# hby1320/pytorch_object_detection

Hardware: AMD Instinct MI355X
Metric: images/sec HISFCOS-R50 640x640 inference (higher is better)
Workload: dtype f32

## Files before the change

pytorch_object_detection_amd/csrc/fd_conv.hip:

```cpp
#include "fd_conv_common.h"

template <int WGM, int WGN, int TM, int TN, bool STEM, bool SB, int TAG, bool SPLIT, bool GATE = false, bool GNS = false, bool H1 = false, bool GEMM = false, bool DUAL = false,
          bool RUP = false>
__global__ __launch_bounds__(WGM * WGN * 64, (TM * TN == 4) ? ((SPLIT || WGM * WGN == 8) ? 2 : (SB ? 3 : 1)) : 1)
void conv_igemm_kernel(ConvArgs a) {
    constexpr int BM = WGM * TM * 32, BN = WGN * TN * 32;
    constexpr int NT = WGM * WGN * 64;
    constexpr int RPP = NT / 8;
    constexpr int AP = BM / RPP, BP = BN / RPP;
    extern __shared__ __attribute__((aligned(16))) char smem[];
    constexpr int NBUF = SB ? 1 : 2;
    float* As = reinterpret_cast<float*>(smem);
    float* Bs = As + NBUF * BM * 32;
    _Float16* Hs = reinterpret_cast<_Float16*>(smem);
    constexpr int HSTG = (BM + BN) * 64;

    const int tid = threadIdx.x, lane = tid & 63, wave = tid >> 6;
    const int wm = wave / WGN, wn = wave % WGN;

    const int nblk = a.mtiles * a.ntiles;
    int bid = blockIdx.x;
    {
        const int q = nblk >> 3, r = nblk & 7, xcd = bid & 7, idx = bid >> 3;
        bid = (xcd < r ? xcd * (q + 1) : r * (q + 1) + (xcd - r) * q) + idx;
    }
    const int mt = bid / a.ntiles, nt = bid - mt * a.ntiles;
    const int m0 = mt * BM, n0 = nt * BN;

    const int lrow = tid >> 3, chunk = tid & 7;
    constexpr unsigned OOB = 0xC0000000u;
    const int esh = (H1 && a.x16) ? 1 : 2;
    const __amdgpu_buffer_rsrc_t xrsrc = __builtin_amdgcn_make_buffer_rsrc((void*)a.x, (short)0, (int)a.x_bytes, 0x00020000);
    const __amdgpu_buffer_rsrc_t wrsrc = __builtin_amdgcn_make_buffer_rsrc((void*)a.w, (short)0, (int)a.w_bytes, 0x00020000);
    unsigned a_off[AP];
    int a_wcs[AP], a_hi0[AP], a_wi0[AP], a_H[AP], a_W[AP];
    const float* g_row[GATE ? AP : 1];
    const long gate_bo = GATE && a.gate_b ? (long)(a.gate_b - a.gate) : 0;
#pragma unroll
    for (int i = 0; i < AP; ++i) {
        const int m = m0 + lrow + RPP * i;
        if (GATE) {
            const int mm = min(m, a.M - 1);
            int sg = 0;
#pragma unroll
            for (int t = 1; t < FD_MAX_SEG; ++t)
                if (t < a.nseg && mm >= a.m_out[t]) sg = t;
            const int img = sg * a.gate_batch + (mm - a.m_out[sg]) / (a.Ho[sg] * a.Wo[sg]);
            g_row[i] = a.gate + (size_t)img * a.gate_cs + chunk * 4;
        }
        if constexpr (GEMM) {
            if (a.is_gemm) {
                a_off[i] = (m < a.M) ? ((unsigned)m * (unsigned)a.x_cs + (unsigned)(a.x_co + chunk * 4)) << esh : OOB;
                a_wcs[i] = 0; a_hi0[i] = 0; a_wi0[i] = 0; a_H[i] = 1; a_W[i] = 1;
                continue;
            }
        }
        if (a.is_gemm) {
            a_off[i] = ((unsigned)m * (unsigned)a.x_cs + (unsigned)(a.x_co + chunk * 4)) << esh;
            a_wcs[i] = 0; a_hi0[i] = 0; a_wi0[i] = 0; a_H[i] = (m < a.M) ? 1 : 0; a_W[i] = 1;
            continue;
        }
        int s = 0;
#pragma unroll
        for (int t = 1; t < FD_MAX_SEG; ++t)
            if (t < a.nseg && m >= a.m_out[t]) s = t;
        const int Ho = a.Ho[s], Wo = a.Wo[s], H = a.H[s], W = a.W[s];
        const int local = m - a.m_out[s];
        const int hw = Ho * Wo;
        const int n = local / hw;
        const int rem = local - n * hw;
        const int ho = rem / Wo, wo = rem - ho * Wo;
        a_hi0[i] = ho * a.stride - a.pad;
        a_wi0[i] = wo * a.stride - a.pad;
        a_H[i] = (m < a.M) ? H : 0;
        a_W[i] = W;
        a_wcs[i] = (W * a.x_cs) << esh;
        a_off[i] = ((unsigned)(a.m_in[s] + n * H * W + a_hi0[i] * W + a_wi0[i]) * (unsigned)a.x_cs +
                    (unsigned)(a.x_co + chunk * 4)) << esh;
        if constexpr (GEMM) { if (m >= a.M) a_off[i] = OOB; }
    }
    unsigned a2_off[DUAL ? AP : 1];
    const __amdgpu_buffer_rsrc_t x2rsrc = __builtin_amdgcn_make_buffer_rsrc((void*)(DUAL ? a.x2 : a.x), (short)0, (int)(DUAL ? a.x2_bytes : 0u), 0x00020000);
    if constexpr (DUAL) {
#pragma unroll
        for (int i = 0; i < AP; ++i) {
            const int m = m0 + lrow + RPP * i;
            const int hw = a.Ho[0] * a.Wo[0];
            const int n = m / hw, rem = m - n * hw;
            const int ho = rem / a.Wo[0], wo = rem - ho * a.Wo[0];
            const unsigned row2 = (unsigned)((n * a.x2_H + ho * a.x2_stride) * a.x2_W + wo * a.x2_stride);
            a2_off[i] = (m < a.M) ? (row2 * (unsigned)a.x2_cs + (unsigned)(a.x2_co + chunk * 4)) * 4u : OOB;
        }
    }
    unsigned b_off[BP];
#pragma unroll
    for (int j = 0; j < BP; ++j) {
        const int n = n0 + lrow + RPP * j;
        b_off[j] = (n < a.Cout && !(H1 && (chunk & 4))) ? ((unsigned)n * (unsigned)a.Kpacked + (unsigned)(chunk * 4)) * 4u : OOB;
    }

    float4 ra[AP], rb[BP], rg[GATE ? AP : 1], rgb[GATE ? AP : 1];
    auto ld_x = [&](unsigned voff, int soff) -> float4 {
        if (H1 && a.x16) {
            const f32x2 v = __builtin_bit_cast(f32x2, __builtin_amdgcn_raw_buffer_load_b64(xrsrc, (int)voff, soff, 0));
            return make_float4(v.x, v.y, 0.f, 0.f);
        }
        return __builtin_bit_cast(float4, __builtin_amdgcn_raw_buffer_load_b128(xrsrc, (int)voff, soff, 0));
    };
    int ld_cc = 0, ld_r = 0, ld_q = 0;
    auto load_tile = [&](int kt) {
        if constexpr (GEMM) {
            const int kb = kt * 128;
            const int kbx = kt << (5 + esh);
            if (GATE) {
#pragma unroll
                for (int i = 0; i < AP; ++i) {
                    rg[i] = *reinterpret_cast<const float4*>(g_row[i] + kt * 32);
                    if (a.gate_b) rgb[i] = *reinterpret_cast<const float4*>(g_row[i] + gate_bo + kt * 32);
                }
            }
            if (DUAL && kt >= a.kt2) {
                const int kb2 = (kt - a.kt2) * 128;
#pragma unroll
                for (int i = 0; i < AP; ++i) ra[i] = __builtin_bit_cast(float4, __builtin_amdgcn_raw_buffer_load_b128(x2rsrc, (int)a2_off[DUAL ? i : 0], kb2, 0));
            } else {
#pragma unroll
                for (int i = 0; i < AP; ++i) ra[i] = ld_x(a_off[i], kbx);
            }
#pragma unroll
            for (int j = 0; j < BP; ++j) rb[j] = __builtin_bit_cast(float4, __builtin_amdgcn_raw_buffer_load_b128(wrsrc, (int)b_off[j], kb, 0));
            return;
        }
        int dr, dq;
        unsigned dbytes;
        bool c_ok = true;
        if (STEM) { dr = kt; dq = 0; dbytes = 0; }
        else {
            dr = ld_r * a.dil;
            dq = ld_q * a.dil;
            dbytes = (unsigned)(dq * a.x_cs + ld_cc * 32) << esh;
            c_ok = ld_cc * 32 + chunk * 4 < a.Cin;
            if (GATE) {
#pragma unroll
                for (int i = 0; i < AP; ++i) {
                    rg[i] = c_ok ? *reinterpret_cast<const float4*>(g_row[i] + ld_cc * 32) : make_float4(0.f, 0.f, 0.f, 0.f);
                    if (a.gate_b) rgb[i] = c_ok ? *reinterpret_cast<const float4*>(g_row[i] + gate_bo + ld_cc * 32) : make_float4(0.f, 0.f, 0.f, 0.f);
                }
            }
            if (++ld_q == a.KW) { ld_q = 0; if (++ld_r * a.KW == a.ntaps) { ld_r = 0; ++ld_cc; } }
        }
#pragma unroll
        for (int i = 0; i < AP; ++i) {
            const int hi = a_hi0[i] + dr, wi = a_wi0[i] + dq + (STEM ? chunk : 0);
            bool ok = (unsigned)hi < (unsigned)a_H[i] && (unsigned)wi < (unsigned)a_W[i] && c_ok;
            if (STEM) ok = ok && (chunk < 7);
            const unsigned off = a_off[i] + (unsigned)__mul24(dr, a_wcs[i]) + dbytes;
            ra[i] = ld_x(ok ? off : OOB, 0);
        }
        const unsigned kb = (unsigned)kt * 128u;
#pragma unroll
        for (int j = 0; j < BP; ++j)
            rb[j] = __builtin_bit_cast(float4, __builtin_amdgcn_raw_buffer_load_b128(wrsrc, (int)(b_off[j] + kb), 0, 0));
    };
    auto store_tile = [&](int buf) {
        if constexpr (SPLIT) {
            _Float16* Ahi = Hs + buf * HSTG;
            _Float16* Alo = Ahi + BM * 32;
            _Float16* Bhi = Alo + BM * 32;
            _Float16* Blo = Bhi + BN * 32;
#pragma unroll
            for (int i = 0; i < AP; ++i) {
                const int row = lrow + RPP * i;
                const f32x4 v = {ra[i].x, ra[i].y, ra[i].z, ra[i].w};
                h4 hi = __builtin_convertvector(v, h4);
                if (H1 && a.x16) hi = fd_h4_bits(ra[i].x, ra[i].y);
                const int off = row * 32 + ((((chunk >> 1) ^ ((row >> 2) & 3)) << 3) | ((chunk & 1) << 2));
                *reinterpret_cast<h4*>(Ahi + off) = hi;
                if constexpr (!H1) {
                    const f32x4 rem = (v - __builtin_convertvector(hi, f32x4)) * FD_SPLIT_SCALE;
                    const h4 lo = __builtin_convertvector(rem, h4);
                    *reinterpret_cast<h4*>(Alo + off) = lo;
                }
            }
#pragma unroll
            for (int j = 0; j < BP; ++j) {
                const int row = lrow + RPP * j;
                if (!H1 || !(chunk & 4)) *reinterpret_cast<float4*>(((chunk & 4) ? Blo : Bhi) + lds_off_h(row, chunk & 3)) = rb[j];
            }
        } else {
#pragma unroll
            for (int i = 0; i < AP; ++i) {
                if (GATE) {
                    if (a.gate_b) {
                        float4 t = make_float4(fmaf(ra[i].x, rg[i].x, rgb[i].x), fmaf(ra[i].y, rg[i].y, rgb[i].y),
                                               fmaf(ra[i].z, rg[i].z, rgb[i].z), fmaf(ra[i].w, rg[i].w, rgb[i].w));
                        if (a.gate_act == FD_ACT_RELU) {
                            t.x = fmaxf(t.x, 0.f); t.y = fmaxf(t.y, 0.f); t.z = fmaxf(t.z, 0.f); t.w = fmaxf(t.w, 0.f);
                        } else if (a.gate_act == FD_ACT_SILU) {
                            t.x *= __builtin_amdgcn_rcpf(1.0f + __expf(-t.x)); t.y *= __builtin_amdgcn_rcpf(1.0f + __expf(-t.y));
                            t.z *= __builtin_amdgcn_rcpf(1.0f + __expf(-t.z)); t.w *= __builtin_amdgcn_rcpf(1.0f + __expf(-t.w));
                        }
                        ra[i] = t;
                    } else { ra[i].x *= rg[i].x; ra[i].y *= rg[i].y; ra[i].z *= rg[i].z; ra[i].w *= rg[i].w; }
                }
                *reinterpret_cast<float4*>(As + buf * BM * 32 + lds_off(lrow + RPP * i, chunk)) = ra[i];
            }
#pragma unroll
            for (int j = 0; j < BP; ++j)
                *reinterpret_cast<float4*>(Bs + buf * BN * 32 + lds_off(lrow + RPP * j, chunk)) = rb[j];
        }
    };

    f32x16 acc[TM][TN];
    f32x16 cor[SPLIT ? TM : 1][SPLIT ? TN : 1];
#pragma unroll
    for (int i = 0; i < TM; ++i)
#pragma unroll
        for (int j = 0; j < TN; ++j)
#pragma unroll
            for (int e = 0; e < 16; ++e) {
                acc[i][j][e] = 0.f;
                if constexpr (SPLIT) cor[i][j][e] = 0.f;
            }

    const int l31 = lane & 31, lh = lane >> 5;
    const int kt0 = blockIdx.y * a.kt_per;
    const int kt1 = min(a.KT, kt0 + a.kt_per);
    if (!STEM) {
        ld_cc = kt0 / a.ntaps;
        const int tap0 = kt0 - ld_cc * a.ntaps;
        ld_r = tap0 / a.KW;
        ld_q = tap0 - ld_r * a.KW;
    }
    float* const ybase = a.y + (size_t)blockIdx.y * a.slice_stride;
    auto mfma_tile = [&](int buf) {
        if constexpr (SPLIT) {
            const _Float16* Ahi = Hs + buf * HSTG + (wm * TM * 32) * 32;
            const _Float16* Alo = Ahi + BM * 32;
            const _Float16* Bhi = Hs + buf * HSTG + 2 * BM * 32 + (wn * TN * 32) * 32;
            const _Float16* Blo = Bhi + BN * 32;
#pragma unroll
            for (int ks = 0; ks < 2; ++ks) {
                h8 ah[TM], al[TM], bh[TN], bl[TN];
#pragma unroll
                for (int i = 0; i < TM; ++i) {
                    ah[i] = *reinterpret_cast<const h8*>(Ahi + lds_off_h(i * 32 + l31, 2 * ks + lh));
                    if constexpr (!H1) al[i] = *reinterpret_cast<const h8*>(Alo + lds_off_h(i * 32 + l31, 2 * ks + lh));
                }
#pragma unroll
                for (int j = 0; j < TN; ++j) {
                    bh[j] = *reinterpret_cast<const h8*>(Bhi + lds_off_h(j * 32 + l31, 2 * ks + lh));
                    if constexpr (!H1) bl[j] = *reinterpret_cast<const h8*>(Blo + lds_off_h(j * 32 + l31, 2 * ks + lh));
                }
#pragma unroll
                for (int i = 0; i < TM; ++i)
#pragma unroll
                    for (int j = 0; j < TN; ++j) {
                        acc[i][j] = __builtin_amdgcn_mfma_f32_32x32x16_f16(ah[i], bh[j], acc[i][j], 0, 0, 0);
                        if constexpr (!H1) {
                            cor[i][j] = __builtin_amdgcn_mfma_f32_32x32x16_f16(ah[i], bl[j], cor[i][j], 0, 0, 0);
                            cor[i][j] = __builtin_amdgcn_mfma_f32_32x32x16_f16(al[i], bh[j], cor[i][j], 0, 0, 0);
                        }
                    }
            }
        } else {
        const float* Ab = As + buf * BM * 32 + (wm * TM * 32) * 32;
            const float* Bb = Bs + buf * BN * 32 + (wn * TN * 32) * 32;
                __builtin_amdgcn_s_setprio(1);
#pragma unroll
            for (int s = 0; s < 4; ++s) {
                float4 fa[TM], fb[TN];
    #pragma unroll
                for (int i = 0; i < TM; ++i) fa[i] = *reinterpret_cast<const float4*>(Ab + lds_off(i * 32 + l31, 2 * s + lh));
    #pragma unroll
                for (int j = 0; j < TN; ++j) fb[j] = *reinterpret_cast<const float4*>(Bb + lds_off(j * 32 + l31, 2 * s + lh));
    #pragma unroll
                for (int i = 0; i < TM; ++i)
    #pragma unroll
                    for (int j = 0; j < TN; ++j) {
                        acc[i][j] = __builtin_amdgcn_mfma_f32_32x32x2f32(fa[i].x, fb[j].x, acc[i][j], 0, 0, 0);
                        acc[i][j] = __builtin_amdgcn_mfma_f32_32x32x2f32(fa[i].y, fb[j].y, acc[i][j], 0, 0, 0);
                        acc[i][j] = __builtin_amdgcn_mfma_f32_32x32x2f32(fa[i].z, fb[j].z, acc[i][j], 0, 0, 0);
                        acc[i][j] = __builtin_amdgcn_mfma_f32_32x32x2f32(fa[i].w, fb[j].w, acc[i][j], 0, 0, 0);
                    }
            }
            __builtin_amdgcn_s_setprio(0);
        }
    };
    load_tile(kt0);
    store_tile(0);
    __syncthreads();
    for (int kt = kt0; kt < kt1 - 1; ++kt) {
        const int buf = SB ? 0 : ((kt - kt0) & 1);
        load_tile(kt + 1);
        mfma_tile(buf);
        if (SB) __syncthreads();
        store_tile(SB ? 0 : (buf ^ 1));
        __syncthreads();
    }
#include "fd_conv_res_prefetch.inc"
    mfma_tile(SB ? 0 : ((kt1 - 1 - kt0) & 1));
    __syncthreads();

#define FD_EPI_RES_PREFETCHED
#include "fd_conv_epilogue.inc"
#undef FD_EPI_RES_PREFETCHED
}

__global__ __launch_bounds__(256) void splitk_reduce_kernel(ConvArgs a, const float* __restrict__ ws, int nslice, int ldw,
                                                             long slab) {
    const int q4 = ldw >> 2;
    const long total = (long)a.M * q4;
    for (long i = (long)blockIdx.x * 256 + threadIdx.x; i < total; i += (long)gridDim.x * 256) {
        const long m = i / q4;
        const int nn = (int)(i - m * q4) * 4;
        float4 v = *reinterpret_cast<const float4*>(ws + m * ldw + nn);
        for (int s = 1; s < nslice; ++s) {
            const float4 u = *reinterpret_cast<const float4*>(ws + s * slab + m * ldw + nn);
            v.x += u.x; v.y += u.y; v.z += u.z; v.w += u.w;
        }
        float o[4] = {v.x, v.y, v.z, v.w};
        float prm = a.seg_param[0];
        if (a.act == FD_ACT_EXP) {
#pragma unroll
            for (int t = 1; t < FD_MAX_SEG; ++t)
                prm = (t < a.nseg && m >= a.m_out[t]) ? a.seg_param[t] : prm;
        }
#pragma unroll
        for (int e = 0; e < 4; ++e) {
            const int n = nn + e;
            if (n >= a.Cout) continue;
            float r = o[e] * (a.scale ? a.scale[n] : 1.0f) + (a.shift ? a.shift[n] : 0.0f);
            const size_t mo = (size_t)out_row(a, (int)m);
            if (a.res) {
                const float rv = a.res16 ? (float)reinterpret_cast<const _Float16*>(a.res)[mo * a.res_cs + a.res_co + n] : a.res[mo * a.res_cs + a.res_co + n];
                r = a.res_mask ? (rv > 0.f ? r : 0.f) : r + rv;
            }
            const float ov = fd_act(r, n >= a.act_c0 ? a.act : FD_ACT_NONE, prm);
            if (a.y16) reinterpret_cast<_Float16*>(a.y)[mo * a.y_cs + a.y_co + n] = (_Float16)ov;
            else a.y[mo * a.y_cs + a.y_co + n] = ov;
        }
    }
}

int fd_launch_splitk_reduce(const ConvArgs& orig, const float* ws, int nslice, int ldw, long slab, hipStream_t stream) {
    long g = ((long)orig.M * (ldw >> 2) + 255) / 256;
    if (g > 16384) g = 16384;
    hipLaunchKernelGGL(splitk_reduce_kernel, dim3((unsigned)g), dim3(256), 0, stream, orig, ws, nslice, ldw, slab);
    FD_CHECK_LAUNCH("fd_conv2d (split-K reduce)");
    return FD_OK;
}

template <int WGM, int WGN, int TM, int TN, bool STEM, bool SB = false, int TAG = 0, bool SPLIT = false, bool GATE = false, bool GNS = false, bool H1 = false, bool GEMM = false,
          bool DUAL = false, bool RUP = false>
static int launch_conv(const ConvArgs& a, hipStream_t stream) {
    constexpr int BM = WGM * TM * 32, BN = WGN * TN * 32;
    constexpr int lds_ab = (SB ? 1 : 2) * (BM + BN) * 32 * 4;
    constexpr int NT = WGM * WGN * 64;
    constexpr int lds_epi = (NT / 64) * 4096;
    constexpr int lds = lds_ab > lds_epi ? lds_ab : lds_epi;
    ConvArgs b = a;
    b.mtiles = (a.M + BM - 1) / BM;
    b.ntiles = (a.Cout + BN - 1) / BN;
    auto kern = conv_igemm_kernel<WGM, WGN, TM, TN, STEM, SB, TAG, SPLIT, GATE, GNS, H1, GEMM, DUAL, RUP>;
    static std::atomic<unsigned> attr_mask{0};
    fd_set_max_lds_once(attr_mask, reinterpret_cast<const void*>(kern), lds);
    hipLaunchKernelGGL(kern, dim3(b.mtiles * b.ntiles, (a.KT + a.kt_per - 1) / a.kt_per), dim3(NT), lds, stream, b);
    FD_CHECK_LAUNCH("fd_conv2d_nhwc_f32");
    return FD_OK;
}

static int dispatch_conv(const fd_conv_params* p, ConvArgs& a, bool stem, hipStream_t stream);

extern "C" int32_t fd_conv_workgroups(const fd_conv_params* p) {
    FD_REQUIRE(p && fd_segs_ok(&p->in) && p->dil >= 1 && p->Cout >= 1, FD_E_INVAL, "fd_conv_workgroups: bad arguments");
    FD_REQUIRE(p->tile == FD_TILE_WINOGRAD4, FD_E_UNSUPPORTED, "fd_conv_workgroups: only FD_TILE_WINOGRAD4 launches can be sliced");
    return fd_wino4_workgroups(p);
}

extern "C" int32_t fd_conv_workgroups_live(const fd_conv_params* p) {
    FD_REQUIRE(p && fd_segs_ok(&p->in) && p->dil >= 1 && p->Cout >= 1, FD_E_INVAL, "fd_conv_workgroups_live: bad arguments");
    FD_REQUIRE(p->tile == FD_TILE_WINOGRAD4, FD_E_UNSUPPORTED, "fd_conv_workgroups_live: only FD_TILE_WINOGRAD4 launches can be sliced");
// ... 29 lines not shown
    if (p->in.nseg > 1)
        FD_REQUIRE(p->stride == 1 && 2 * p->pad == p->dil * (p->KH - 1) && p->KH == p->KW, FD_E_INVAL,
                   "fd_conv2d: multi-level input needs stride 1 and 'same' padding");

    FD_REQUIRE(p->res_mode >= 0 && p->res_mode <= 2, FD_E_INVAL, "fd_conv2d: res_mode %d", p->res_mode);
    if (p->res && p->res_mode == 2) {
        FD_REQUIRE(p->tile == FD_TILE_AUTO || p->tile == FD_TILE_64x64 || p->tile == FD_TILE_128x64_SB || p->tile == FD_TILE_64x128_SB, FD_E_UNSUPPORTED,
                   "fd_conv2d: res_mode 2 is built for tiles 64x64, 128x64_SB, 64x128_SB (got %d)", p->tile);
        FD_REQUIRE(!stem && p->KH == 1 && p->KW == 1 && p->stride == 1 && p->pad == 0 && p->in.nseg == 1 && p->Cin % 32 == 0 && p->precision == FD_PREC_F32 &&
                       p->ksplit <= 1 && p->sc_H <= 0 && p->out_H <= 0 && p->out_W <= 0 && !p->gate && !p->gn_stats && !p->x2 && p->tag != 1 &&
                       p->in.H[0] % 2 == 0 && p->in.W[0] % 2 == 0 && p->Cout % 4 == 0 && p->y_cs % 4 == 0 && p->y_co % 4 == 0 && ((uintptr_t)p->y & 15) == 0 &&
                       p->res_cs % 4 == 0 && p->res_co % 4 == 0 && ((uintptr_t)p->res & 15) == 0,
                   FD_E_UNSUPPORTED, "fd_conv2d: res_mode 2 (half-resolution addend) needs an fp32 1x1 stride-1 unpadded single-level conv with even H, W, Cin %% 32 == 0, "
                                     "16-byte views, no split-K / scatter / gate / gn_stats / x2 / tag 1");
    }
    FD_REQUIRE(p->wg_count <= 0 || p->tile == FD_TILE_WINOGRAD4, FD_E_UNSUPPORTED, "fd_conv2d: wg_first / wg_count (a slice of the layer's grid) exist for FD_TILE_WINOGRAD4 only");
    FD_REQUIRE(p->sk_wgs <= 0 || p->tile == FD_TILE_WINOGRAD4, FD_E_UNSUPPORTED, "fd_conv2d: sk_wgs (the persistent stream-K form) exists for FD_TILE_WINOGRAD4 only");
    FD_REQUIRE(!p->io_f16 || (p->tile != FD_TILE_WINOGRAD && p->tile != FD_TILE_WINOGRAD4 && p->tile != FD_TILE_NARROW), FD_E_UNSUPPORTED,
               "fd_conv2d: io_f16 (f16 activation maps) is built for the FD_PREC_F16 implicit-GEMM tiles only");
    if (p->tile == FD_TILE_WINOGRAD) return fd_launch_conv_wino(p, stream);
    if (p->tile == FD_TILE_WINOGRAD4) return fd_launch_conv_wino4(p, stream);
    if (p->tile == FD_TILE_NARROW) return fd_launch_conv_narrow(p, stream);

    ConvArgs a;
    a.x16 = a.y16 = a.res16 = 0;
    a.x = p->x; a.w = p->w; a.scale = p->scale; a.shift = p->shift; a.res = p->res; a.y = p->y;
    a.x_cs = p->x_cs; a.x_co = p->x_co; a.res_cs = p->res_cs; a.res_co = p->res_co; a.y_cs = p->y_cs; a.y_co = p->y_co;
    a.Cin = p->Cin; a.Cout = p->Cout; a.KW = p->KW; a.stride = p->stride; a.pad = p->pad; a.dil = p->dil;
    a.act = p->act; a.act_c0 = p->act_c0;
    a.res_mask = (p->res && p->res_mode == 1) ? 1 : 0;
    a.res_up = 0;
    a.nseg = p->in.nseg;
    long mo = 0;
    for (int s = 0; s < FD_MAX_SEG; ++s) {
        if (s < p->in.nseg) {
            a.H[s] = p->in.H[s]; a.W[s] = p->in.W[s];
            a.Ho[s] = (p->in.H[s] + 2 * p->pad - p->dil * (p->KH - 1) - 1) / p->stride + 1;
            a.Wo[s] = (p->in.W[s] + 2 * p->pad - p->dil * (p->KW - 1) - 1) / p->stride + 1;
            if (p->out_H > 0 || p->out_W > 0) {
                FD_REQUIRE(p->in.nseg == 1 && p->out_H > 0 && p->out_W > 0, FD_E_INVAL, "fd_conv2d: out_H / out_W need a single-level input");
                a.Ho[s] = p->out_H; a.Wo[s] = p->out_W;
            }
            FD_REQUIRE(a.Ho[s] >= 1 && a.Wo[s] >= 1, FD_E_INVAL, "fd_conv2d: empty output");
            a.m_in[s] = p->in.m_start[s];
            a.m_out[s] = (int)mo;
            mo += (long)p->in.batch * a.Ho[s] * a.Wo[s];
        } else {
            a.H[s] = a.W[s] = a.Ho[s] = a.Wo[s] = 1; a.m_in[s] = 0; a.m_out[s] = (int)mo;
        }
        a.seg_param[s] = p->seg_param[s];
    }
    a.m_out[FD_MAX_SEG] = (int)mo;
    FD_REQUIRE(mo > 0 && mo < (1L << 31), FD_E_INVAL, "fd_conv2d: row count out of range");
    a.M = (int)mo;
    a.sc_on = 0; a.sc_sy = a.sc_sx = 1; a.sc_oy = a.sc_ox = 0; a.sc_H = a.sc_W = 0;
    long y_rows = mo;
    if (p->sc_H > 0) {
        FD_REQUIRE(p->in.nseg == 1 && !stem && p->sc_W > 0 && p->sc_sy >= 1 && p->sc_sx >= 1 && p->sc_oy >= 0 && p->sc_ox >= 0 &&
                       p->sc_sy * (a.Ho[0] - 1) + p->sc_oy < p->sc_H && p->sc_sx * (a.Wo[0] - 1) + p->sc_ox < p->sc_W,
                   FD_E_INVAL, "fd_conv2d: output scatter does not fit its %d x %d target", p->sc_H, p->sc_W);
        a.sc_on = 1; a.sc_sy = p->sc_sy; a.sc_sx = p->sc_sx; a.sc_oy = p->sc_oy; a.sc_ox = p->sc_ox; a.sc_H = p->sc_H; a.sc_W = p->sc_W;
        y_rows = (long)p->in.batch * p->sc_H * p->sc_W;
    }
    FD_REQUIRE((long)p->in.m_start[p->in.nseg] * p->x_cs < (1L << 31) && y_rows * p->y_cs < (1L << 31), FD_E_UNSUPPORTED,
               "fd_conv2d: tensor exceeds 2^31 elements");
    if (stem) { a.KT = 7; a.ntaps = 7; a.Kpacked = 7 * 32; }
    else { const int cch = (p->Cin + 31) / 32; a.ntaps = p->KH * p->KW; a.KT = a.ntaps * cch; a.Kpacked = a.ntaps * cch * 32; }
    a.mtiles = a.ntiles = 0;

    a.vec_epi = (p->Cout % 4 == 0 && p->y_cs % 4 == 0 && p->y_co % 4 == 0 && ((uintptr_t)p->y & 15) == 0 &&
                 (!p->res || (p->res_cs % 4 == 0 && p->res_co % 4 == 0 && ((uintptr_t)p->res & 15) == 0)))
                    ? 1 : 0;

    a.is_gemm = (!stem && p->KH == 1 && p->KW == 1 && p->stride == 1 && p->pad == 0) ? 1 : 0;
    {
        const long xb = (long)p->in.m_start[p->in.nseg] * p->x_cs * 4, wb = (long)p->Cout * a.Kpacked * 4;
        FD_REQUIRE(xb < 0xC0000000L && wb < 0xC0000000L, FD_E_UNSUPPORTED, "fd_conv2d: input / weight buffer exceeds 3 GiB");
        a.x_bytes = (unsigned)xb; a.w_bytes = (unsigned)wb;
        for (int sg = 0; sg < p->in.nseg; ++sg)
            FD_REQUIRE((long)p->in.W[sg] * p->x_cs * 4 < (1L << 23), FD_E_UNSUPPORTED, "fd_conv2d: image row of %ld bytes exceeds the 24-bit row-stride path", (long)p->in.W[sg] * p->x_cs * 4);
    }
    a.Cout_epi = a.Cout; a.kt_per = a.KT; a.slice_stride = 0;
    a.p_halo = 0;
    a.x2 = nullptr; a.x2_cs = a.x2_co = 0; a.x2_stride = 1; a.x2_H = a.x2_W = 1; a.kt2 = 0; a.x2_bytes = 0;
    if (p->x2) {
        FD_REQUIRE(!stem && p->KH == 1 && p->KW == 1 && p->pad == 0 && p->stride == 1 && p->in.nseg == 1 && p->Cin % 32 == 0 && p->x2_Cin >= 32 && p->x2_Cin % 32 == 0 &&
                       p->precision == FD_PREC_F32 && p->ksplit <= 1 && !a.sc_on && p->out_H <= 0 && !p->gate && !p->gn_stats && p->tag != 1,
                   FD_E_UNSUPPORTED, "fd_conv2d: `x2` needs an fp32 1x1 stride-1 unpadded single-level conv with Cin, x2_Cin multiples of 32, no split-K / scatter / gate / gn_stats");
        FD_REQUIRE(p->x2_stride >= 1 && p->x2_cs % 4 == 0 && p->x2_co % 4 == 0 && p->x2_cs >= p->x2_co + p->x2_Cin && ((uintptr_t)p->x2 & 15) == 0 &&
                       (p->in.H[0] - 1) * p->x2_stride < p->x2_H && (p->in.W[0] - 1) * p->x2_stride < p->x2_W,
                   FD_E_INVAL, "fd_conv2d: `x2` view must be 16-byte addressable and cover the strided samples of a %d x %d output", p->in.H[0], p->in.W[0]);
        const long x2b = (long)p->in.batch * p->x2_H * p->x2_W * p->x2_cs * 4;
        FD_REQUIRE(x2b < 0xC0000000L, FD_E_UNSUPPORTED, "fd_conv2d: `x2` buffer exceeds 3 GiB");
        a.x2 = p->x2; a.x2_cs = p->x2_cs; a.x2_co = p->x2_co; a.x2_stride = p->x2_stride; a.x2_H = p->x2_H; a.x2_W = p->x2_W;
        a.kt2 = p->Cin / 32; a.x2_bytes = (unsigned)x2b;
        a.KT = (p->Cin + p->x2_Cin) / 32; a.Kpacked = a.KT * 32; a.kt_per = a.KT;
        a.w_bytes = (unsigned)((long)p->Cout * a.Kpacked * 4);
        switch (p->tile) {
            case FD_TILE_64x128_SB: return launch_conv<2, 2, 1, 2, false, true, 0, false, false, false, false, true, true>(a, stream);
            case FD_TILE_64x64: return launch_conv<2, 2, 1, 1, false, false, 0, false, false, false, false, true, true>(a, stream);
            case FD_TILE_128x128_SB: return launch_conv<2, 2, 2, 2, false, true, 0, false, false, false, false, true, true>(a, stream);
            case FD_TILE_AUTO: case FD_TILE_128x64_SB: return launch_conv<2, 2, 2, 1, false, true, 0, false, false, false, false, true, true>(a, stream);
            default: fd_set_error("fd_conv2d: `x2` is built for tiles 64x64, 128x64_SB, 64x128_SB, 128x128_SB (got %d)", p->tile); return FD_E_UNSUPPORTED;
        }
    }
    if (p->io_f16) {
        FD_REQUIRE(p->precision == FD_PREC_F16 && !stem && !p->gate && !p->gn_stats && !p->x2 && (p->io_f16 & ~7) == 0 && p->tile != FD_TILE_WAVE64 && p->tile != FD_TILE_128x128_PATCH,
                   FD_E_UNSUPPORTED, "fd_conv2d: io_f16 (f16 activation maps) needs FD_PREC_F16 on the plain conv tiles, no gate / gn_stats / x2");
        FD_REQUIRE(a.vec_epi || !(p->io_f16 & 6), FD_E_UNSUPPORTED, "fd_conv2d: f16 output / residual maps need 4-channel aligned views (Cout, y_cs, y_co, res_cs, res_co multiples of 4)");
        FD_REQUIRE(!(p->io_f16 & 4) || p->res, FD_E_INVAL, "fd_conv2d: io_f16 names an f16 residual but res is NULL");
        a.x16 = p->io_f16 & 1; a.y16 = (p->io_f16 >> 1) & 1; a.res16 = (p->io_f16 >> 2) & 1;
        if (a.x16) a.x_bytes = (unsigned)((long)p->in.m_start[p->in.nseg] * p->x_cs * 2);
    }
    if (p->tile == FD_TILE_F16K64) return fd_launch_conv_f16k64(p, a, stream);
    a.gate = nullptr; a.gate_cs = 0; a.gate_hw = 1; a.gate_b = nullptr; a.gate_act = FD_ACT_NONE; a.gate_batch = p->in.batch;
    a.gn_stats = nullptr; a.gn_G = 1; a.gn_cg = 4;
    if (p->gn_stats) {
        FD_REQUIRE(p->gn_groups >= 1 && p->Cout % p->gn_groups == 0 && (p->Cout / p->gn_groups) % 4 == 0 && 32 % (p->Cout / p->gn_groups) == 0 &&
                       p->Cout % 32 == 0 && a.vec_epi && !a.sc_on && p->ksplit <= 1 && p->precision == FD_PREC_F32 && ((uintptr_t)p->gn_stats & 7) == 0,
                   FD_E_UNSUPPORTED, "fd_conv2d: gn_stats needs fp32, Cout %% 32 == 0, 4 | Cout / groups | 32, 16-byte output views, no split-K / scatter");
        a.gn_stats = p->gn_stats; a.gn_G = p->gn_groups; a.gn_cg = p->Cout / p->gn_groups;
    }
    if (p->gate) {
        FD_REQUIRE(a.is_gemm && p->precision == FD_PREC_F32 && p->ksplit <= 1 && !a.sc_on && p->out_H <= 0 && !p->gn_stats, FD_E_UNSUPPORTED,
                   "fd_conv2d: `gate` needs an fp32 1x1 stride-1 unpadded conv, no split-K / scatter / gn_stats");
        FD_REQUIRE(p->gate_cs >= p->Cin && p->gate_cs % 4 == 0 && ((uintptr_t)p->gate & 15) == 0, FD_E_INVAL, "fd_conv2d: gate rows must be 16-byte aligned, gate_cs >= Cin");
        FD_REQUIRE(!p->gate_b || ((((uintptr_t)p->gate_b) & 15) == 0 && (p->gate_act == FD_ACT_NONE || p->gate_act == FD_ACT_RELU || p->gate_act == FD_ACT_SILU)),
                   FD_E_INVAL, "fd_conv2d: gate_b must be 16-byte aligned, gate_act in {NONE, RELU, SILU}");
        a.gate = p->gate; a.gate_cs = p->gate_cs; a.gate_hw = p->in.H[0] * p->in.W[0];
        a.gate_b = p->gate_b; a.gate_act = p->gate_b ? p->gate_act : FD_ACT_NONE;
        if (p->gate_b && a.Cout > 64 && (long)((a.M + 63) / 64) * ((a.Cout + 127) / 128) >= 512) {
            if (p->Cin % 32 == 0 && !a.sc_on) return launch_conv<2, 2, 1, 2, false, true, 0, false, true, false, false, true>(a, stream);
            return launch_conv<2, 2, 1, 2, false, true, 0, false, true>(a, stream);
        }
        if (a.Cout <= 32) return launch_conv<4, 1, 1, 1, false, false, 0, false, true>(a, stream);
        const long m128 = (a.M + 127) / 128;
        if (a.Cout <= 64) {
            if (m128 < 512) return launch_conv<2, 2, 1, 1, false, false, 0, false, true>(a, stream);
            return launch_conv<2, 2, 2, 1, false, false, 0, false, true>(a, stream);
        }
        if (a.Cout <= 96 && m128 >= 512) return launch_conv<4, 1, 1, 3, false, false, 0, false, true>(a, stream);
        if (m128 * ((a.Cout + 127) / 128) < 640) return launch_conv<2, 2, 1, 2, false, false, 0, false, true>(a, stream);
        return launch_conv<2, 2, 2, 2, false, false, 0, false, true>(a, stream);
    }
    if (p->tile == FD_TILE_WAVE64) {
        FD_REQUIRE(a.is_gemm && p->Cin % 32 == 0 && p->Cout % 32 == 0 && p->precision == FD_PREC_F32 && p->ksplit <= 1 && !a.sc_on && p->out_H <= 0 &&
                       a.vec_epi && !p->gate && p->act_c0 % 32 == 0 && (p->act == FD_ACT_NONE || p->act == FD_ACT_RELU || p->act == FD_ACT_SILU),
                   FD_E_UNSUPPORTED, "fd_conv2d: FD_TILE_WAVE64 needs an fp32 1x1 stride-1 unpadded conv with Cin, Cout, act_c0 multiples of 32, 16-byte output "
                   "views, ReLU / SiLU / no activation, no split-K / scatter / gate");
        FD_REQUIRE(p->w_frag && ((uintptr_t)p->w_frag & 15) == 0, FD_E_UNSUPPORTED, "fd_conv2d: FD_TILE_WAVE64 needs fd_conv_params.w_frag (fd_pack_conv_weight_wave_f32)");
        return fd_launch_conv_wave(a, p->w_frag, stream);
    }
    if (p->tile == FD_TILE_128x128_PATCH) {
        int wmax = 0;
        for (int sg = 0; sg < p->in.nseg; ++sg) wmax = p->in.W[sg] > wmax ? p->in.W[sg] : wmax;
        FD_REQUIRE(!stem && p->KH == 3 && p->KW == 3 && p->stride == 1 && p->pad == p->dil && p->ksplit <= 1 && !a.sc_on && !p->gn_stats &&
                       p->out_H <= 0 && FD_PATCH_BM + 2 * p->dil * (wmax + 1) <= FD_PATCH_MAXROWS,
                   FD_E_UNSUPPORTED, "fd_conv2d: FD_TILE_128x128_PATCH needs a 3x3 stride-1 'same' conv with 128 + 2*dil*(W+1) <= %d rows (W=%d dil=%d)",
                   FD_PATCH_MAXROWS, wmax, p->dil);
        a.p_halo = p->dil * (wmax + 1);
        return fd_launch_conv_patch(a, p->tag == 1, p->precision == FD_PREC_F16X3, stream);
    }

    const int ksplit = p->ksplit > 1 ? p->ksplit : 1;
    if (ksplit > 1) {
        FD_REQUIRE(!stem && ksplit <= 64 && a.KT >= ksplit, FD_E_INVAL, "fd_conv2d: ksplit=%d needs 1 < ksplit <= min(64, K-tiles=%d)", ksplit, a.KT);
        const ConvArgs orig = a;
        const int ldw = (a.Cout + 3) & ~3;
        const long slab = (long)a.M * ldw;
        FD_REQUIRE(p->workspace && ((uintptr_t)p->workspace & 15) == 0 && p->workspace_bytes >= (int64_t)ksplit * slab * 4, FD_E_INVAL,
                   "fd_conv2d: split-K needs a 16-byte aligned workspace of fd_conv_workspace_bytes() bytes");
        a.kt_per = (a.KT + ksplit - 1) / ksplit;
        a.y = (float*)p->workspace; a.y_cs = ldw; a.y_co = 0; a.slice_stride = slab; a.Cout_epi = ldw;
        a.scale = a.shift = a.res = nullptr; a.act = FD_ACT_NONE; a.vec_epi = 1; a.sc_on = 0;
        a.y16 = a.res16 = 0;
        const int rc = dispatch_conv(p, a, stem, stream);
        if (rc != FD_OK) return rc;
        return fd_launch_splitk_reduce(orig, (const float*)p->workspace, (a.KT + a.kt_per - 1) / a.kt_per, ldw, slab, stream);
    }
    return dispatch_conv(p, a, stem, stream);
}

static int dispatch_conv(const fd_conv_params* p, ConvArgs& a, bool stem, hipStream_t stream) {

    if (stem) { FD_REQUIRE(!a.gn_stats, FD_E_UNSUPPORTED, "fd_conv2d: gn_stats on the stem"); return launch_conv<2, 2, 2, 1, true>(a, stream); }
    if (p->precision == FD_PREC_F16X3) {
        FD_REQUIRE(!stem, FD_E_UNSUPPORTED, "fd_conv2d: the stem runs in exact fp32 only");
        const bool tg = p->tag == 1;
        switch (p->tile) {
            case FD_TILE_AUTO:
                if (a.Cout <= 32) return launch_conv<4, 1, 1, 1, false, false, 0, true>(a, stream);
                if (a.Cout <= 64) return launch_conv<2, 2, 1, 1, false, false, 0, true>(a, stream);
                if (a.Cout <= 96) return launch_conv<4, 1, 1, 3, false, false, 0, true>(a, stream);
                return launch_conv<2, 2, 1, 2, false, false, 0, true>(a, stream);
            case FD_TILE_128x128:
                return tg ? launch_conv<2, 2, 2, 2, false, false, 1, true>(a, stream) : launch_conv<2, 2, 2, 2, false, false, 0, true>(a, stream);
            case FD_TILE_128x128_SB:
                return tg ? launch_conv<2, 2, 2, 2, false, true, 1, true>(a, stream) : launch_conv<2, 2, 2, 2, false, true, 0, true>(a, stream);
            case FD_TILE_128x64: return launch_conv<2, 2, 2, 1, false, false, 0, true>(a, stream);
            case FD_TILE_64x128: return launch_conv<2, 2, 1, 2, false, false, 0, true>(a, stream);
            case FD_TILE_64x64: return launch_conv<2, 2, 1, 1, false, false, 0, true>(a, stream);
            case FD_TILE_128x64_SB: return launch_conv<2, 2, 2, 1, false, true, 0, true>(a, stream);
            case FD_TILE_64x128_SB: return launch_conv<2, 2, 1, 2, false, true, 0, true>(a, stream);
            case FD_TILE_128x32: return launch_conv<4, 1, 1, 1, false, false, 0, true>(a, stream);
            case FD_TILE_128x96: return launch_conv<4, 1, 1, 3, false, false, 0, true>(a, stream);
            case FD_TILE_128x96_SB: return launch_conv<4, 1, 1, 3, false, true, 0, true>(a, stream);
            case FD_TILE_256x128:
                return tg ? launch_conv<4, 2, 2, 2, false, false, 1, true>(a, stream) : launch_conv<4, 2, 2, 2, false, false, 0, true>(a, stream);
            case FD_TILE_256x128_SB:
                return tg ? launch_conv<4, 2, 2, 2, false, true, 1, true>(a, stream) : launch_conv<4, 2, 2, 2, false, true, 0, true>(a, stream);
            default: fd_set_error("fd_conv2d: tile id %d has no split-f16 kernel", p->tile); return FD_E_UNSUPPORTED;
        }
    }
    if (p->precision == FD_PREC_F16) {
        FD_REQUIRE(!a.gn_stats && !a.gate, FD_E_UNSUPPORTED, "fd_conv2d: FD_PREC_F16 has no gn_stats / gate form");
        auto blocks = [&](int bm, int bn) { return (long)((a.M + bm - 1) / bm) * ((a.Cout + bn - 1) / bn); };
        switch (p->tile) {
            case FD_TILE_AUTO:
                if (a.Cout <= 32) return launch_conv<4, 1, 1, 1, false, false, 0, true, false, false, true>(a, stream);
                if (a.Cout <= 64) return blocks(128, 64) >= 512 ? launch_conv<2, 2, 2, 1, false, false, 0, true, false, false, true>(a, stream)
                                                                : launch_conv<2, 2, 1, 1, false, false, 0, true, false, false, true>(a, stream);
                if (a.Cout <= 96) return launch_conv<4, 1, 1, 3, false, false, 0, true, false, false, true>(a, stream);
                if (blocks(128, 128) >= 512) return launch_conv<2, 2, 2, 2, false, false, 0, true, false, false, true>(a, stream);
                if (blocks(64, 128) >= 256) return launch_conv<2, 2, 1, 2, false, false, 0, true, false, false, true>(a, stream);
                return launch_conv<2, 2, 1, 1, false, false, 0, true, false, false, true>(a, stream);
            case FD_TILE_128x128: return launch_conv<2, 2, 2, 2, false, false, 0, true, false, false, true>(a, stream);
            case FD_TILE_128x128_SB: return launch_conv<2, 2, 2, 2, false, true, 0, true, false, false, true>(a, stream);
            case FD_TILE_128x64: return launch_conv<2, 2, 2, 1, false, false, 0, true, false, false, true>(a, stream);
            case FD_TILE_64x128: return launch_conv<2, 2, 1, 2, false, false, 0, true, false, false, true>(a, stream);
            case FD_TILE_64x64: return launch_conv<2, 2, 1, 1, false, false, 0, true, false, false, true>(a, stream);
            case FD_TILE_128x32: return launch_conv<4, 1, 1, 1, false, false, 0, true, false, false, true>(a, stream);
            case FD_TILE_128x96: return launch_conv<4, 1, 1, 3, false, false, 0, true, false, false, true>(a, stream);
            default: fd_set_error("fd_conv2d: tile id %d has no f16 kernel", p->tile); return FD_E_UNSUPPORTED;
        }
    }
    FD_REQUIRE(p->precision == FD_PREC_F32, FD_E_INVAL, "fd_conv2d: unknown precision %d", p->precision);
    if (p->tag == 1) {
        switch (p->tile) {
            case FD_TILE_128x128: return launch_conv<2, 2, 2, 2, false, false, 1>(a, stream);
            case FD_TILE_128x128_SB: return launch_conv<2, 2, 2, 2, false, true, 1>(a, stream);
            case FD_TILE_64x128_SB: return launch_conv<2, 2, 1, 2, false, true, 1>(a, stream);
            case FD_TILE_128x64_SB: return launch_conv<2, 2, 2, 1, false, true, 1>(a, stream);
            default: break;
        }
    }
    if (a.gn_stats) {
        if (a.is_gemm && p->Cin % 32 == 0 && !a.sc_on) {
            switch (p->tile) {
                case FD_TILE_64x128_SB: return launch_conv<2, 2, 1, 2, false, true, 0, false, false, true, false, true>(a, stream);
                case FD_TILE_AUTO: case FD_TILE_128x64_SB: return launch_conv<2, 2, 2, 1, false, true, 0, false, false, true, false, true>(a, stream);
                default: break;
            }
        }
        switch (p->tile) {
            case FD_TILE_64x64: return launch_conv<2, 2, 1, 1, false, false, 0, false, false, true>(a, stream);
            case FD_TILE_128x64: return launch_conv<2, 2, 2, 1, false, false, 0, false, false, true>(a, stream);
            case FD_TILE_64x128: return launch_conv<2, 2, 1, 2, false, false, 0, false, false, true>(a, stream);
            case FD_TILE_64x128_SB: return launch_conv<2, 2, 1, 2, false, true, 0, false, false, true>(a, stream);
            case FD_TILE_AUTO: case FD_TILE_128x64_SB: return launch_conv<2, 2, 2, 1, false, true, 0, false, false, true>(a, stream);
            default: fd_set_error("fd_conv2d: gn_stats is built for tiles 64x64, 128x64(_SB), 64x128(_SB), WAVE64 and WINOGRAD (got %d)", p->tile); return FD_E_UNSUPPORTED;
        }
    }
    if (p->res && p->res_mode == 2) {
        FD_REQUIRE(a.is_gemm && p->in.nseg == 1 && p->Cin % 32 == 0 && p->precision == FD_PREC_F32 && p->ksplit <= 1 && !a.sc_on && p->out_H <= 0 && !p->gate &&
                       !p->gn_stats && !p->x2 && a.vec_epi && p->tag != 1 && p->in.H[0] % 2 == 0 && p->in.W[0] % 2 == 0,
                   FD_E_UNSUPPORTED, "fd_conv2d: res_mode 2 (half-resolution addend) needs an fp32 1x1 stride-1 unpadded single-level conv with even H, W, Cin %% 32 == 0, "
                                     "16-byte views, no split-K / scatter / gate / gn_stats / x2");
// ... 50 lines not shown
```

pytorch_object_detection_amd/csrc/fd_conv_common.h:

```cpp
#pragma once
#include "fd_common.h"

typedef float f32x16 __attribute__((ext_vector_type(16)));
typedef float f32x4 __attribute__((ext_vector_type(4)));
typedef _Float16 h4 __attribute__((ext_vector_type(4)));
typedef _Float16 h8 __attribute__((ext_vector_type(8)));
#define FD_SPLIT_SCALE 2048.0f

struct ConvArgs {
    const float* x; const float* w; const float* scale; const float* shift; const float* res; float* y;
    int x_cs, x_co, res_cs, res_co, y_cs, y_co;
    int Cin, Cout, KW, stride, pad, dil, act, act_c0;
    int M, KT, ntaps, Kpacked;
    int nseg;
    int H[FD_MAX_SEG], W[FD_MAX_SEG], Ho[FD_MAX_SEG], Wo[FD_MAX_SEG];
    int m_in[FD_MAX_SEG];
    int m_out[FD_MAX_SEG + 1];
    float seg_param[FD_MAX_SEG];
    int mtiles, ntiles;
    int vec_epi;
    int is_gemm;
    int Cout_epi;
    int kt_per;
    long slice_stride;
    unsigned x_bytes, w_bytes;
    int res_mask;
    int res_up;
    int sc_on, sc_sy, sc_sx, sc_oy, sc_ox, sc_H, sc_W;
    const float* gate; int gate_cs, gate_hw;
    const float* gate_b; int gate_act, gate_batch;
    float* gn_stats; int gn_G, gn_cg;
    const float* x2; int x2_cs, x2_co, x2_stride, x2_H, x2_W, kt2; unsigned x2_bytes;
    int p_halo;
    int x16, y16, res16;
    int wide8;
};

__device__ __forceinline__ float4 fd_ld_h4(const void* p) {
    const h4 v = *reinterpret_cast<const h4*>(p);
    return make_float4((float)v[0], (float)v[1], (float)v[2], (float)v[3]);
}
typedef float f32x2 __attribute__((ext_vector_type(2)));
__device__ __forceinline__ h4 fd_h4_bits(float lo, float hi) {
    const f32x2 t = {lo, hi};
    return __builtin_bit_cast(h4, t);
}
__device__ __forceinline__ void fd_st_h4(void* p, const float4& v) {
    const f32x4 f = {v.x, v.y, v.z, v.w};
    *reinterpret_cast<h4*>(p) = __builtin_convertvector(f, h4);
}

#define FD_PATCH_BM 128
#define FD_PATCH_MAXROWS 320
int fd_launch_conv_patch(const ConvArgs& a, int tag, int split, hipStream_t stream);
int fd_launch_conv_wino(const fd_conv_params* p, hipStream_t stream);
int fd_launch_conv_wino4(const fd_conv_params* p, hipStream_t stream);
int fd_wino4_workgroups(const fd_conv_params* p);
int fd_wino4_workgroups_live(const fd_conv_params* p, int first, int count);
int fd_launch_conv_narrow(const fd_conv_params* p, hipStream_t stream);
int fd_launch_conv_wave(const ConvArgs& a, const float* wfrag, hipStream_t stream);
int fd_launch_conv_f16k64(const fd_conv_params* p, ConvArgs& a, hipStream_t stream);
int fd_launch_splitk_reduce(const ConvArgs& orig, const float* ws, int nslice, int ldw, long slab, hipStream_t stream);

__device__ __forceinline__ long out_row(const ConvArgs& a, int m) {
    if (!a.sc_on) return m;
    const int hw = a.Ho[0] * a.Wo[0];
    const int n = m / hw, rem = m - n * hw;
    const int i = rem / a.Wo[0], j = rem - i * a.Wo[0];
    return ((long)n * a.sc_H + (a.sc_sy * i + a.sc_oy)) * a.sc_W + (a.sc_sx * j + a.sc_ox);
}

__device__ __forceinline__ long res_row_up(const ConvArgs& a, int m) {
    const int W = a.Wo[0], hw = a.Ho[0] * W;
    const int n = m / hw, rem = m - n * hw;
    const int i = rem / W, j = rem - i * W;
    return ((long)n * (a.Ho[0] >> 1) + (i >> 1)) * (W >> 1) + (j >> 1);
}

__device__ __forceinline__ void wave_lds_sync() {
    __builtin_amdgcn_fence(__ATOMIC_RELEASE, "wavefront");
    __builtin_amdgcn_s_waitcnt(0xc07f);
    __builtin_amdgcn_wave_barrier();
    __builtin_amdgcn_fence(__ATOMIC_ACQUIRE, "wavefront");
}

__device__ __forceinline__ float fd_quad_xor1(float v) { return __builtin_bit_cast(float, __builtin_amdgcn_mov_dpp(__builtin_bit_cast(int, v), 0xB1, 0xF, 0xF, true)); }
__device__ __forceinline__ float fd_quad_xor2(float v) { return __builtin_bit_cast(float, __builtin_amdgcn_mov_dpp(__builtin_bit_cast(int, v), 0x4E, 0xF, 0xF, true)); }

__device__ __forceinline__ void fd_gn_rowstats(float* gn_stats, int gn_G, int gn_cg, const float4& v, size_t m, int nn, int lane, bool ok) {
    float s1 = (v.x + v.y) + (v.z + v.w);
    float s2 = (v.x * v.x + v.y * v.y) + (v.z * v.z + v.w * v.w);
    const int cgq = gn_cg >> 2;
    if (cgq > 1) { s1 += fd_quad_xor1(s1); s2 += fd_quad_xor1(s2); }
    if (cgq > 2) { s1 += fd_quad_xor2(s1); s2 += fd_quad_xor2(s2); }
    if (cgq > 4) { s1 += __shfl_xor(s1, 4); s2 += __shfl_xor(s2, 4); }
    if (ok && ((lane & 7) & (cgq - 1)) == 0)
        reinterpret_cast<float2*>(gn_stats)[m * gn_G + nn / gn_cg] = make_float2(s1, s2);
}

__device__ __forceinline__ int lds_off(int row, int chunk) { return row * 32 + ((chunk ^ ((row >> 1) & 7)) << 2); }
__device__ __forceinline__ int lds_off_h(int row, int c8) { return row * 32 + ((c8 ^ ((row >> 2) & 3)) << 3); }

__device__ __forceinline__ void fd_wino4_pack_one(const float* __restrict__ w, const float* __restrict__ scale, float* __restrict__ out,
                                                  int N, int K, int mode, int n, int k) {
    const double G[6][3] = {{0.25, 0.0, 0.0}, {-1.0 / 6, -1.0 / 6, -1.0 / 6}, {-1.0 / 6, 1.0 / 6, -1.0 / 6},
                            {1.0 / 24, 1.0 / 12, 1.0 / 6}, {1.0 / 24, -1.0 / 12, 1.0 / 6}, {0.0, 0.0, 1.0}};
    double gg[3][3];
#pragma unroll
    for (int r = 0; r < 3; ++r)
#pragma unroll
        for (int c = 0; c < 3; ++c) {
            double v = 0.0;
            if (n < N) {
                if (mode == 0) v = w[((long)n * K + k) * 9 + r * 3 + c];
                else v = (double)w[((long)k * N + n) * 9 + (2 - r) * 3 + (2 - c)] * (scale ? (double)scale[k] : 1.0);
            }
            gg[r][c] = v;
        }
// ... 48 lines not shown
```

Measured before the change: 1419.

## Use precomputed tap offsets and validity bitmasks for implicit-GEMM A loads

Adds a tap-table path to the implicit-GEMM conv kernel. For each row it precomputes a bitmask of which kernel taps fall inside the image. It also builds a per-tap byte-offset table in the kernel args and biases the buffer resource base so padded offsets stay non-negative. This removes the per-iteration hi/wi bounds arithmetic and the tap/channel counter logic from the load loop, replacing it with a mask test and the buffer-load soffset. The cost is larger kernel args, extra registers for the masks, and two instantiated k-loop variants.

```diff
diff --git a/pytorch_object_detection_amd/csrc/fd_conv.hip b/pytorch_object_detection_amd/csrc/fd_conv.hip
--- a/pytorch_object_detection_amd/csrc/fd_conv.hip
+++ b/pytorch_object_detection_amd/csrc/fd_conv.hip
@@ -30,9 +30,12 @@
     const int lrow = tid >> 3, chunk = tid & 7;
     constexpr unsigned OOB = 0xC0000000u;
     const int esh = (H1 && a.x16) ? 1 : 2;
-    const __amdgpu_buffer_rsrc_t xrsrc = __builtin_amdgcn_make_buffer_rsrc((void*)a.x, (short)0, (int)a.x_bytes, 0x00020000);
+    const bool use_tap = !STEM && !GEMM && !GATE && a.tap;
+    const unsigned x_bias = use_tap ? a.tap_bias : 0u;
+    const __amdgpu_buffer_rsrc_t xrsrc = __builtin_amdgcn_make_buffer_rsrc((void*)((const char*)a.x - x_bias), (short)0, (int)(a.x_bytes + x_bias), 0x00020000);
     const __amdgpu_buffer_rsrc_t wrsrc = __builtin_amdgcn_make_buffer_rsrc((void*)a.w, (short)0, (int)a.w_bytes, 0x00020000);
     unsigned a_off[AP];
+    unsigned a_mask[AP];
     int a_wcs[AP], a_hi0[AP], a_wi0[AP], a_H[AP], a_W[AP];
     const float* g_row[GATE ? AP : 1];
     const long gate_bo = GATE && a.gate_b ? (long)(a.gate_b - a.gate) : 0;
@@ -58,6 +61,7 @@
         if (a.is_gemm) {
             a_off[i] = ((unsigned)m * (unsigned)a.x_cs + (unsigned)(a.x_co + chunk * 4)) << esh;
             a_wcs[i] = 0; a_hi0[i] = 0; a_wi0[i] = 0; a_H[i] = (m < a.M) ? 1 : 0; a_W[i] = 1;
+            a_mask[i] = (m < a.M) ? 1u : 0u;
             continue;
         }
         int s = 0;
@@ -78,6 +82,16 @@
         a_off[i] = ((unsigned)(a.m_in[s] + n * H * W + a_hi0[i] * W + a_wi0[i]) * (unsigned)a.x_cs +
                     (unsigned)(a.x_co + chunk * 4)) << esh;
         if constexpr (GEMM) { if (m >= a.M) a_off[i] = OOB; }
+        a_mask[i] = 0;
+        if (use_tap) {
+            a_off[i] = ((unsigned)(a.m_in[s] + n * H * W + ho * a.stride * W + wo * a.stride) * (unsigned)a.x_cs + (unsigned)(a.x_co + chunk * 4)) << esh;
+            unsigned cols = 0, msk = 0;
+#pragma clang loop vectorize(disable) unroll(disable)
+            for (int q = 0; q < a.KW; ++q) cols |= ((unsigned)(a_wi0[i] + q * a.dil) < (unsigned)W ? 1u : 0u) << q;
+#pragma clang loop vectorize(disable) unroll(disable)
+            for (int r = 0, sh = 0; sh < a.ntaps; ++r, sh += a.KW) msk |= ((unsigned)(a_hi0[i] + r * a.dil) < (unsigned)H ? cols : 0u) << sh;
+            a_mask[i] = (m < a.M) ? msk : 0u;
+        }
     }
     unsigned a2_off[DUAL ? AP : 1];
     const __amdgpu_buffer_rsrc_t x2rsrc = __builtin_amdgcn_make_buffer_rsrc((void*)(DUAL ? a.x2 : a.x), (short)0, (int)(DUAL ? a.x2_bytes : 0u), 0x00020000);
@@ -161,6 +175,19 @@
 #pragma unroll
         for (int j = 0; j < BP; ++j)
             rb[j] = __builtin_bit_cast(float4, __builtin_amdgcn_raw_buffer_load_b128(wrsrc, (int)(b_off[j] + kb), 0, 0));
+    };
+    int tp_t = 0, tp_cc = 0;
+    unsigned tp_off = 0;
+    auto load_tile_tap = [&](int kt) {
+        const int soff = (int)tp_off + (tp_cc << (5 + esh));
+        const unsigned tbit = (tp_cc * 32 + chunk * 4 < a.Cin) ? 1u << tp_t : 0u;
+        if (++tp_t == a.ntaps) { tp_t = 0; ++tp_cc; }
+        tp_off = a.tap_off[tp_t];
+#pragma unroll
+        for (int i = 0; i < AP; ++i) ra[i] = ld_x((a_mask[i] & tbit) ? a_off[i] : OOB, soff);
+        const int kb = kt * 128;
+#pragma unroll
+        for (int j = 0; j < BP; ++j) rb[j] = __builtin_bit_cast(float4, __builtin_amdgcn_raw_buffer_load_b128(wrsrc, (int)b_off[j], kb, 0));
     };
     auto store_tile = [&](int buf) {
         if constexpr (SPLIT) {
@@ -231,6 +258,7 @@
         const int tap0 = kt0 - ld_cc * a.ntaps;
         ld_r = tap0 / a.KW;
         ld_q = tap0 - ld_r * a.KW;
+        tp_cc = ld_cc; tp_t = tap0; tp_off = a.tap_off[tap0 & 31];
     }
     float* const ybase = a.y + (size_t)blockIdx.y * a.slice_stride;
     auto mfma_tile = [&](int buf) {
@@ -287,17 +315,21 @@
             __builtin_amdgcn_s_setprio(0);
         }
     };
-    load_tile(kt0);
-    store_tile(0);
-    __syncthreads();
-    for (int kt = kt0; kt < kt1 - 1; ++kt) {
-        const int buf = SB ? 0 : ((kt - kt0) & 1);
-        load_tile(kt + 1);
-        mfma_tile(buf);
-        if (SB) __syncthreads();
-        store_tile(SB ? 0 : (buf ^ 1));
+    auto k_loop = [&](auto& load) {
+        load(kt0);
+        store_tile(0);
         __syncthreads();
-    }
+        for (int kt = kt0; kt < kt1 - 1; ++kt) {
+            const int buf = SB ? 0 : ((kt - kt0) & 1);
+            load(kt + 1);
+            mfma_tile(buf);
+            if (SB) __syncthreads();
+            store_tile(SB ? 0 : (buf ^ 1));
+            __syncthreads();
+        }
+    };
+    if (use_tap) k_loop(load_tile_tap);
+    else k_loop(load_tile);
 #include "fd_conv_res_prefetch.inc"
     mfma_tile(SB ? 0 : ((kt1 - 1 - kt0) & 1));
     __syncthreads();
@@ -493,6 +525,7 @@
     }
     a.Cout_epi = a.Cout; a.kt_per = a.KT; a.slice_stride = 0;
     a.p_halo = 0;
+    a.tap = 0; a.tap_bias = 0;
     a.x2 = nullptr; a.x2_cs = a.x2_co = 0; a.x2_stride = 1; a.x2_H = a.x2_W = 1; a.kt2 = 0; a.x2_bytes = 0;
     if (p->x2) {
         FD_REQUIRE(!stem && p->KH == 1 && p->KW == 1 && p->pad == 0 && p->stride == 1 && p->in.nseg == 1 && p->Cin % 32 == 0 && p->x2_Cin >= 32 && p->x2_Cin % 32 == 0 &&
@@ -592,8 +625,22 @@
     return dispatch_conv(p, a, stem, stream);
 }
 
+static void fd_conv_tap_setup(const fd_conv_params* p, ConvArgs& a, bool stem) {
+    a.tap = 0; a.tap_bias = 0;
+    const bool one_by_one = p->KH == 1 && p->KW == 1 && p->pad == 0;
+    if (stem || a.gate || a.ntaps > 32 || (a.nseg > 1 && !one_by_one)) return;
+    const int esh = a.x16 ? 1 : 2;
+    const long W = a.W[0], px = (long)a.x_cs << esh;
+    const long bias = one_by_one ? 0 : ((long)p->pad * W + p->pad) * px;
+    const long last = (((long)(p->KH - 1) * W + (p->KW - 1)) * p->dil) * px + ((long)(a.KT / a.ntaps - 1) << (5 + esh));
+    if (last >= (long)a.x_bytes + bias || last >= (1L << 30) || (long)a.x_bytes + bias >= 0xC0000000L) return;
+    for (int r = 0; r < p->KH; ++r)
+        for (int q = 0; q < p->KW; ++q) a.tap_off[r * p->KW + q] = (unsigned)((((long)r * W + q) * p->dil) * px);
+    a.tap = 1; a.tap_bias = (unsigned)bias;
+}
+
 static int dispatch_conv(const fd_conv_params* p, ConvArgs& a, bool stem, hipStream_t stream) {
-
+    fd_conv_tap_setup(p, a, stem);
     if (stem) { FD_REQUIRE(!a.gn_stats, FD_E_UNSUPPORTED, "fd_conv2d: gn_stats on the stem"); return launch_conv<2, 2, 2, 1, true>(a, stream); }
     if (p->precision == FD_PREC_F16X3) {
         FD_REQUIRE(!stem, FD_E_UNSUPPORTED, "fd_conv2d: the stem runs in exact fp32 only");
diff --git a/pytorch_object_detection_amd/csrc/fd_conv_common.h b/pytorch_object_detection_amd/csrc/fd_conv_common.h
--- a/pytorch_object_detection_amd/csrc/fd_conv_common.h
+++ b/pytorch_object_detection_amd/csrc/fd_conv_common.h
@@ -34,6 +34,7 @@
     int p_halo;
     int x16, y16, res16;
     int wide8;
+    int tap; unsigned tap_bias; unsigned tap_off[32];
 };
 
 __device__ __forceinline__ float4 fd_ld_h4(const void* p) {
```

Result: no change. 1421, median of 6 (+0.1%).
